# tphakala/birdnet-go

Measured on AMD Instinct MI355X. Metric: 3s-48kHz clips/sec (whole node) + max-abs prob diff vs TFLite, BirdNET v2.4, higher is better.
Workload: dtype f32; 1 GPU; BASELINE configs[1]: BirdNET v2.4 fp32, batch 256 x 3 s @ 48 kHz per GPU, mel front-end + CNN + head on device, raw logits out; batch_per_gpu=256, n_samples=144000, n_classes=6522, pipeline_depth=2, input_sets=4

## Files before the change

### birdnet-go_amd/csrc/engine.cpp

```cpp
#include "engine.h"

#include <algorithm>
#include <cmath>
#include <cstdio>
#include <cstdlib>
#include <cstring>
#include <mutex>
#include <sstream>

#include "../../include/bnhip.h"
#include "hostpipe.h"

namespace bnhip {

#define HIPCHK(call)                                                                           \
    do {                                                                                       \
        hipError_t e_ = (call);                                                                \
        if (e_ != hipSuccess) {                                                                \
            *err = std::string(#call) + ": " + hipGetErrorString(e_);                          \
            return false;                                                                      \
        }                                                                                      \
    } while (0)

Engine::~Engine() {
// ... 49 lines not shown
        if (steps[si].kind == S_FRONTEND) {
            specs[steps[si].spec].G = reinterpret_cast<const double*>(steps[si].w0);
            specs[steps[si].spec].window = steps[si].w1;
        }
        if (steps[si].kind == S_STFT) {
            specs[steps[si].spec].window_full = steps[si].w0;
            specs[steps[si].spec].bins = reinterpret_cast<const int*>(steps[si].w1);
            specs[steps[si].spec].stft_tw = reinterpret_cast<const double*>(steps[si].w2);
        }
    }
    HIPCHK(hipMalloc((void**)&d_stage_in, (size_t)max_batch * n_samples * 4));
    HIPCHK(hipMalloc((void**)&d_stage_logits, (size_t)max_batch * n_classes * 4));
    HIPCHK(hipMalloc((void**)&d_post_conf, (size_t)max_batch * n_classes * 4));
    if (emb_dim) HIPCHK(hipMalloc((void**)&d_stage_emb, (size_t)max_batch * emb_dim * 4));
    if (!defer_weights) mark_bf16_storage();
    if (autotune && !defer_weights) tune_or_load();
    *code = BNHIP_OK;
    return true;
}

namespace {
struct DevStreams { hipStream_t k[Engine::kMaxKStreams] = {nullptr, nullptr, nullptr, nullptr}; hipStream_t xfer = nullptr; int refs = 0; };
std::mutex g_ds_mu;
std::map<int, DevStreams> g_ds;
}

hipStream_t Engine::kernel_stream(int i) {
    if (i < 0 || i >= kMaxKStreams || device < 0) return nullptr;
    if (kstream[i]) return kstream[i];
    std::lock_guard<std::mutex> lk(g_ds_mu);
    DevStreams& ds = g_ds[device];
// ... 43 lines not shown
            if (!ctx_stream[c]) { ctx_stream[c] = kernel_stream(1 + c); if (!ctx_stream[c]) { *err = "hipStreamCreate failed"; return false; } }
            if (!ev_ctx_done[c]) HIPCHK(hipEventCreateWithFlags(&ev_ctx_done[c], hipEventDisableTiming));
        }
        if (!ctx_arena[c]) {
            if (c == 0) ctx_arena[c] = act_arena;
            else HIPCHK(hipMalloc((void**)&ctx_arena[c], std::max<size_t>(act_bytes, 256)));
        }
    }
    return true;
}

void Engine::finish_deferred() {
    if (device < 0) return;
    hipSetDevice(device);
    mark_bf16_storage();
    if (autotune) tune_or_load();
    defer_weights = false;
}

PwParams Engine::pw_params(const Step& s, int n, bool lane_tuning) const {
    PwParams p{nullptr, s.w0, s.w1, nullptr, nullptr, nullptr, n * s.H * s.W, s.Co, s.C, s.H * s.W, s.act, lane_tuning ? s.nt : s.nt_full,
               lane_tuning ? s.wm : s.wm_full};
    p.prec = precision; p.sw = pw_sw;
    p.a_bf16 = vals[s.in0].half ? 1 : 0; p.out_bf16 = vals[s.out].half ? 1 : 0;
    p.res_bf16 = (s.in2 >= 0 && vals[s.in2].half) ? 1 : 0;
    return p;
}
PwTail tail_of(const Step& s, const Step& c) {
    PwTail t;
    t.kind = s.tail; t.H = s.H; t.W = s.W;
    if (s.tail == 2) { t.k = c.kh; t.pt = c.pt; t.pl = c.pl; t.act = c.act; t.w = c.w0; t.bias = c.w1; }
// ... 19 lines not shown
        const Step& a = steps[si]; const Step& b = steps[si + 1];
        if (a.kind == S_MINMAX && b.kind == S_NORMALIZE && a.in0 == v_input && b.in0 == v_input && b.in1 == a.out) { norm_pair = si; break; }
    }
    if (norm_pair < 0 || !clip_norm_resident_fits(n_samples)) { norm_pair = -1; return; }
    pcm_direct = true;
    for (int si = 0; si < (int)steps.size(); si++) {
        if (si == norm_pair || si == norm_pair + 1) continue;
        const Step& s = steps[si];
        if (s.in0 == v_input || s.in1 == v_input || s.in2 == v_input) pcm_direct = false;
    }
}
bool Engine::norm_resident_taken(int n, const void* x, int bits, const float* xn) const {
    if (norm_pair < 0 || n <= 16) return false;
    const uintptr_t in_align = bits == 16 ? 8 : bits == 24 ? 4 : 16;
    return !(reinterpret_cast<uintptr_t>(x) & (in_align - 1)) && !(reinterpret_cast<uintptr_t>(xn) & 15);
}

float* Engine::vptr(int v, const float* d_in, float* d_logits, float* d_emb, int lane) const {
    if (v < 0) return nullptr;
    if (v == v_input) return const_cast<float*>(d_in);
    if (v == v_logits) return d_logits;
    if (part_hand && v == v_hand) return part_hand;
    (void)d_emb;
    char* base = cur_arena ? cur_arena : act_arena;
    if (lane >= 0) return reinterpret_cast<float*>(base + (size_t)lane * lane_bytes + vals[v].offset_lane);
    return reinterpret_cast<float*>(base + vals[v].offset);
}

hipEvent_t Engine::get_event() {
    if (!ev_pool.empty()) { hipEvent_t e = ev_pool.back(); ev_pool.pop_back(); return e; }
// ... 209 lines not shown
    for (int si = part_s0; si < s_end; si++) {
      for (int li = 0; li < nl; li++) {
        const Step& s = steps[si];
        const float* d_in = lanes[li].d_in; float* d_logits = lanes[li].d_logits; float* d_emb = lanes[li].d_emb;
        const int n = lanes[li].n, clip0 = nl > 1 ? li : -1;
        hipStream_t stream = lanes[li].st;
        float* in0 = vptr(s.in0, d_in, d_logits, d_emb, clip0);
        float* in1 = vptr(s.in1, d_in, d_logits, d_emb, clip0);
        float* in2 = vptr(s.in2, d_in, d_logits, d_emb, clip0);
        float* out = vptr(s.out, d_in, d_logits, d_emb, clip0);
        float* out2 = vptr(s.out2, d_in, d_logits, d_emb, clip0);
        if (s.kind == S_DW && si > 0 && steps[si - 1].tail == 2 && tail_taken(si - 1, n, nl > 1)) continue;
        if (s.kind == S_MEAN_PARTIAL && si > 0 && steps[si - 1].tail == 1 && tail_taken(si - 1, n, nl > 1)) continue;
        if (s.kind == S_MEAN_FINISH && si > 1 && steps[si - 2].tail == 1 && tail_taken(si - 2, n, nl > 1)) continue;
        if (s.kind == S_NORMALIZE && si == norm_pair + 1 && res_x[li]) continue;
        ProfEntry pe{};
        static const char* dbg_sync_before = getenv("BNHIP_DEBUG_SYNC_BEFORE");
        static const char* dbg_sync_after = getenv("BNHIP_DEBUG_SYNC_AFTER");
        static const char* dbg_ctx1_only = getenv("BNHIP_DEBUG_CTX1_ONLY");
        if (dbg_ctx1_only && cur_ctx == 1 && !strstr(dbg_ctx1_only, s.kclass)) continue;
        static const char* dbg_ctx1_skip = getenv("BNHIP_DEBUG_CTX1_SKIP");
        if (dbg_ctx1_skip && cur_ctx == 1 && strstr(dbg_ctx1_skip, s.kclass)) continue;
        if (dbg_sync_before && (!strcmp(dbg_sync_before, s.kclass) || s.name.rfind(dbg_sync_before, 0) == 0)) hipStreamSynchronize(stream);
        const bool prof_this = profiling && (profile_filter.empty() || profile_filter == s.kclass);
        if (prof_this) { pe.a = get_event(); pe.b = get_event(); pe.step = si; pe.n = n; hipEventRecord(pe.a, stream); }
        switch (s.kind) {
            case S_MINMAX:
                if (si == norm_pair && res_x[li]) {
                    const WinView lane_win = win_at(pcm.win, lanes[li].clip0);
                    if (!launch_clip_norm_resident(res_x[li], res_bits[li], n, n_samples, specs[0].eps, specs[0].norm_sub, specs[0].norm_mul,
// ... 79 lines not shown
                if (p.wm >= 13) p.wm = 10;
                if (p.wm >= 5 && s.wbx) launch_pw_bx3(p, s.wbx, stream);
                else launch_pw_gemm(p, stream);
                break;
            }
            case S_DW: {
                DwParams p = dw_params(s, in0, out, n);
                p.in_bf16 = vals[s.in0].half ? 1 : 0; p.out_bf16 = vals[s.out].half ? 1 : 0;
                if (s.dwl) launch_dwconv_lds(p, out2, s.shape, stream);
                else launch_dwconv(p, out2, stream);
                break;
            }
            case S_EXPAND_DW:
                {
                    StemGeom sg{s.H2, s.W2, s.pt2, s.pl2};
                    launch_expand_dw(in0, s.w0, s.w1, s.w2, s.w3, out, out2, n, s.H, s.W, s.C, s.Co,
                                     s.Ho, s.Wo, s.kh, s.sh, s.pt, s.pl, s.act, s.act2, s.shape, s.mode == 1 ? &sg : nullptr, stream,
                                     s.bx ? s.wbx : nullptr, precision, vals[s.out].half ? 1 : 0, vals[s.in0].half ? 1 : 0);
                }
                break;
            case S_MEAN_PARTIAL:
                launch_mean_partial(in0, out, n, s.H * s.W, s.C, s.S, stream);
                break;
            case S_MEAN_FINISH:
                launch_mean_finish(in0, out, n, s.H * s.W, s.C, s.S, stream);
                break;
            case S_SE: {
                SeParams p{in0, s.S, s.H * s.W, s.w0, s.w1, s.w2, s.w3, out, n, s.C, s.Cr, s.act, s.act2};
                if (cur_stream) p.threads = 256;
                launch_se(p, stream);
                break;
            }
            case S_UNARY:
// ... 176 lines not shown
```

### birdnet-go_amd/csrc/engine.h

```cpp
#pragma once
#include <hip/hip_runtime.h>

#include <map>
#include <string>
#include <vector>

#include "kernels.h"
#include "tflite_model.h"

namespace bnhip {

enum StepKind { S_MINMAX, S_FRONTEND, S_NORMALIZE, S_STFT, S_MELFIN, S_MELBAND, S_CONV_DIRECT, S_PW, S_DW, S_EXPAND_DW, S_MEAN_PARTIAL, S_MEAN_FINISH, S_SE, S_UNARY, S_BINARY,
                S_EW_UNARY, S_EW_BINARY, S_POOL, S_COPY, S_SOFTMAX, S_REDUCE, S_CONV_GENERIC,
                S_CONV_IGEMM };

struct GenGeom {
    int d[4] = {1, 1, 1, 1};
    long sa[4] = {0, 0, 0, 0}, sb[4] = {0, 0, 0, 0}, so[4] = {0, 0, 0, 0};
    long offa = 0, offo = 0;
    bool a_const = false, b_const = false;
    int mask = 0;
    float alpha = 0.f;
    bool fill = false;
    int dh = 1, dw = 1, depthwise = 0, mult = 1;
// ... 81 lines not shown
    int pw_sw = 0;
    bool use_graphs = false;
    void drop_graphs();
    static constexpr int kMaxDepth = 3;
    int depth = 1;
    hipStream_t ctx_stream[kMaxDepth] = {nullptr, nullptr, nullptr};
    char* ctx_arena[kMaxDepth] = {nullptr, nullptr, nullptr};
    static constexpr int kMinMaxScratch = 16 * (2 * kMinMaxParts + 2);
    float* mm_scratch = nullptr;
    bool mm_dirty = false;
    bool norm_resident = true;
    int norm_pair = -1;
    bool pcm_direct = false;
    void find_norm_pair();
    bool norm_resident_taken(int n, const void* x, int bits, const float* xn) const;
    hipEvent_t ev_ctx_fork = nullptr, ev_ctx_done[kMaxDepth] = {nullptr, nullptr, nullptr};
    unsigned call_idx = 0;
    bool run_pipelined(const float* d_in, int n, float* d_logits, float* d_emb, std::string* err);
    void sync_contexts();
    int host_depth = 2;
    bool ensure_contexts(int d, std::string* err, bool with_streams = true);
    bool run_on_context(int c, hipStream_t st, const float* d_in, int n, float* d_logits, float* d_emb, std::string* err, PcmSource pcm = {});
    int split_step = -1, v_hand = -1;
    float* d_hand = nullptr;
    std::vector<int> split_candidates;
    void pick_split();
    size_t hand_clip_bytes() const { return v_hand < 0 ? 0 : vals[v_hand].elems * (vals[v_hand].half ? 2 : 4); }
    bool ensure_hand(std::string* err);
    bool run_part(int c, hipStream_t st, int s0, int s1, const float* d_in, int n, float* hand, float* d_logits, float* d_emb, std::string* err, PcmSource pcm = {});
    int heatmap_pruned_step() const;
// ... 86 lines not shown
```

### birdnet-go_amd/csrc/expdw.hip

```cpp
#include "kernels.h"
#include "pw_common.h"

#include <algorithm>
#include <type_traits>
#include <cmath>
#include <cstdio>
#include <cstdlib>
#include <cstring>
#include <vector>

namespace bnhip {

struct ExpDwParams {
    const float* x; const float* we; const float* be; const float* wd; const float* bd;
    float* y; float* partial;
    int B, H, W, Cin, Cmid, Ho, Wo, pt, pl, act_e, act_d, tiles_h, tiles_w, cchunks, Kw, Cp;
    int Hin = 0, Win = 0, pts = 0, pls = 0;
    const uint16_t* wep = nullptr; int Kp = 0;
    int prec = 0;
    int xsh = 0, xsw = 1, ysh = 0, ysw = 1, tr = 0;
    int in_bf16 = 0, out_bf16 = 0;
    FDiv d_bpc{}, d_cch{}, d_tw{};
    int cpp = 0;
    FDiv d_part{};
};
#define ED_ES 36
#define ED_PERM2 0xfdce5764b98a1320ull
#define ED_PERM4 0xfdce9ba875461320ull
__device__ __forceinline__ int ed_perm(unsigned long long magic, int lane) {
    return (int)((magic >> ((lane >> 2) * 4)) & 15ull) * 4 + (lane & 3);
}
constexpr bool ed_perm_c4_rule(unsigned long long magic) {
    for (int g = 0; g < 16; g++)
        if (((magic >> (4 * g)) & 1ull) != (unsigned long long)((g >> 1) & 1)) return false;
    return true;
}
constexpr int expdw_min_waves(int K, int S, int TOW, int TRH) {
    const int tiw = (TOW - 1) * S + K, jt = (TRH * tiw + 15) / 16, jtw = (jt + 3) / 4;
    return jtw <= 4 ? 4 : (jtw == 5 ? 3 : 2);
// ... 340 lines not shown
            }
        }
    }
    if (tid < K * K * 8) wds[tid] = wdreg;
    __syncthreads();
    }

    const float4 sum = ed_phase2<K, S, TOH, TOW, TRH, 4>(p, E, wds, b, oh0, ow0, vr0, vr1, wave, tx, c4, n_base, bv, [] {});
    if (p.partial) {
        ed_sums_lanes(sum, red, wave, lane, c4);
        __syncthreads();
        ed_sums_out(p, red, tid, (size_t)b * tiles + tile, n_base);
    }
}

template <int K, int S, int TOH, int TOW, int TRH, bool STEM, int KW, bool LOOP = !STEM, int NW = 4, int PH = 0, int NS = 1>
__global__ __launch_bounds__(64 * NW, expdw_sk_waves(K, S, TOH, TOW, TRH, PH == 1 ? 16 * NS : KW, !LOOP, NW)) void k_expand_dw_sk(ExpDwParams p, unsigned nblk) {
    static_assert(PH == 0 || PH == 1, "phase 1 on the f32 or on the bf16 pipe");
    constexpr bool B16 = PH == 1;
    static_assert(!B16 || (LOOP && !STEM), "bf16 phase 1: chunk-loop form");
    static_assert(NS == 1 || B16, "several resident slabs: bf16 operands only");
    constexpr int KP = 32 * NS;
    static_assert(PH != 1 || KW == 24 || KW == 32, "one-product form: layers of the bf16 engines");
    static_assert(NW == 4 || (NW == 8 && LOOP && TOH % 8 == 0), "eight-wave blocks: chunk-loop form, tile height a multiple of 8");
    static_assert(KW == 16 || KW == 24 || KW == 32, "one or two K slabs, or a slab and a half");
    static_assert(!STEM || KW == 24, "the stem's window is 3 rows x 4 columns x 2 channels");
    constexpr int TIH = (TOH - 1) * S + K, TIW = (TOW - 1) * S + K;
    static_assert(TRH <= TIH, "TRH is a cap on the footprint rows");
    constexpr int NPIX = TRH * TIW, NPIXP = (NPIX + 15) / 16 * 16;
    constexpr int JT = NPIXP / 16, JTW = (JT + NW - 1) / NW;
    constexpr int SW = TOW / 8;
    constexpr int NMMA = B16 ? 2 * NS : KW / 2;
    __shared__ __attribute__((aligned(16))) float lds[NPIX * ED_ES + 64 * NW + K * K * 32];
// ... 31 lines not shown
    const int jtv = (nvalid + 15) >> 4;
    const int Cin = p.Cin;
    const int ncc = LOOP ? min(cpp, p.cchunks - cc0) : 1;
    const size_t tile_index = (size_t)b * tiles + tile;

    static_assert(SW * S == 2 || SW * S == 4, "lane permutation tables cover SW*S in {2, 4}");
    constexpr unsigned long long PERM = SW * S == 2 ? ED_PERM2 : ED_PERM4;
    const int pl = ed_perm(PERM, lane);
    const int c4 = pl & 7, tx = pl >> 3;

    bool xin[JTW];
    f32x4 xA[B16 ? 1 : JTW];
    f32x4 xB[(KW == 32 && !B16) ? JTW : 1];
    f32x2 xH[(KW == 24 && !B16) ? JTW : 1];
    bf16x8 xb[B16 ? JTW : 1][NS];
    auto load_x = [&]() {
        const float* xbase = STEM ? p.x + (size_t)b * p.Hin * p.Win * 2 : p.x;
#pragma unroll
        for (int a = 0; a < JTW; a++) {
            const int j = 16 * (wave + NW * a) + li;
            const int r = j / TIW, c = j - r * TIW;
            const int iw = iw0 + c;
            xin[a] = j < nvalid && iw >= 0 && iw < p.W;
            const int ihc = min(ih0 + vr0 + r, p.H - 1), iwc = min(max(iw, 0), p.W - 1);
            if constexpr (STEM) {
                const int row0 = ihc * 2 - p.pts, col0 = iwc * 2 - p.pls;
                auto tap2 = [&](int row, int col) {
                    const bool v = row >= 0 && row < p.Hin && col >= 0 && col < p.Win;
                    const float2 u = *reinterpret_cast<const float2*>(xbase + ((size_t)min(max(row, 0), p.Hin - 1) * p.Win + min(max(col, 0), p.Win - 1)) * 2);
                    return (f32x2){v ? u.x : 0.f, v ? u.y : 0.f};
                };
                const f32x2 u = tap2(row0 + (kq >> 1), col0 + (kq & 1) * 2), w = tap2(row0 + (kq >> 1), col0 + (kq & 1) * 2 + 1);
// ... 181 lines not shown
        }
        if (tid < K * K * 8) wds[tid] = q.wd;
        const float4 bv = q.bv;
        __syncthreads();
        if (LOOP && ci + 1 < ncc) fetch(cc + 1, q);

        const float4 sum = ed_phase2<K, S, TOH, TOW, TRH, NW>(p, E, wds, b, oh0, ow0, vr0, vr1, wave, tx, c4, n_base, bv, land);
        if (p.partial) ed_sums_lanes(sum, red, wave, lane, c4);
    }
    if (p.partial) {
        __syncthreads();
        ed_sums_out<NW>(p, red, tid, tile_index, (cc0 + ncc - 1) * 32);
    }
}

int expdw_kw(int Cin) { return (Cin & 1) ? (Cin + 15) / 16 * 16 : (Cin + 7) / 8 * 8; }
int expdw_skw(int Cin, int act_e, bool stem) {
    const int kw = expdw_kw(Cin);
    return !stem && act_e == ACT_SWISH && (kw == 16 || kw == 24 || kw == 32) ? kw : 0;
}
int expdw_cp(int Cmid) { return (Cmid + 31) / 32 * 32; }
struct ExpDwShape { int k, s, toh, tow, trh, nw = 4; };
static const ExpDwShape kExpDwShapes[] = {
    {3, 1, 8, 16, 10}, {3, 1, 4, 16, 6}, {3, 1, 8, 32, 6}, {3, 1, 8, 32, 10},
    {5, 1, 8, 16, 12}, {5, 1, 4, 16, 8}, {5, 1, 8, 32, 6}, {5, 1, 12, 16, 12},
    {3, 2, 4, 8, 9}, {3, 2, 8, 8, 12}, {3, 2, 8, 8, 17},
    {5, 2, 4, 8, 11}, {5, 2, 4, 16, 6}, {5, 2, 8, 8, 19},
    {3, 1, 8, 16, 10, 8}, {3, 1, 8, 32, 6, 8}, {3, 1, 8, 32, 10, 8}, {5, 1, 8, 16, 12, 8}, {5, 1, 8, 32, 6, 8},
    {3, 2, 8, 8, 12, 8}, {3, 2, 8, 8, 17, 8}, {5, 2, 8, 8, 19, 8},
};
// ... 90 lines not shown
        }
    return img;
}
bool expdw_sk_pipe16(int Cin, int act_e, bool stem, int prec, bool have_image) {
    static const bool off = getenv("BNHIP_EXPDW_B16") && atoi(getenv("BNHIP_EXPDW_B16")) == 0;
    static const int max_ns = getenv("BNHIP_EXPDW_B16_NS") ? atoi(getenv("BNHIP_EXPDW_B16_NS")) : 5;
    if (off || !have_image || stem || act_e != ACT_SWISH || !expdw_bx_ok(Cin)) return false;
    const int kw = expdw_skw(Cin, act_e, stem), ns = expdw_kp(Cin) / 32;
    return prec == 1 && ((kw == 24 || kw == 32) || (kw == 0 && (ns == 2 || ns == 3 || ns == 5) && ns <= max_ns));
}
bool expdw_supported(int k, int s, int Cin, int Cmid, int act_e, int prec) {
    if (!((k == 3 || k == 5) && (s == 1 || s == 2) && (Cin & 3) == 0 && (Cmid & 3) == 0)) return false;
    if (Cin <= 128) return true;
    return prec == 1 && expdw_sk_pipe16(Cin, act_e, false, prec, true);
}
template <int K, int S, int TH, int TW, int TR, bool H8, bool BX>
static void ed_launch(const ExpDwParams& p, unsigned nblk, hipStream_t st, bool fullw) {
    constexpr int VW = expdw_fullw_vw(K, S, TW);
    if constexpr (VW > 0) {
        if (fullw) {
            hipLaunchKernelGGL((k_expand_dw<K, S, TH, TW, TR, H8, BX, false, VW>), dim3(nblk), dim3(256), 0, st, p, nblk);
            return;
        }
    }
    hipLaunchKernelGGL((k_expand_dw<K, S, TH, TW, TR, H8, BX>), dim3(nblk), dim3(256), 0, st, p, nblk);
}
void launch_expand_dw(const float* x, const float* we, const float* be, const float* wd, const float* bd, float* y,
                      float* partial, int B, int H, int W, int Cin, int Cmid, int Ho, int Wo, int k, int s, int pt,
                      int pl, int act_e, int act_d, int shape, const StemGeom* stem, hipStream_t st, const uint16_t* wep, int prec, int out_bf16,
                      int in_bf16) {
    const bool pipe16 = expdw_sk_pipe16(Cin, act_e, stem != nullptr, prec, wep != nullptr);
    const ExpDwGeo g0{k, s, H, W, Ho, Wo, pt, pl, stem != nullptr, pipe16 ? 0 : expdw_skw(Cin, act_e, stem != nullptr)};
    if (!expdw_shape_fits(shape, g0, false)) shape = expdw_default_shape(g0);
    if (shape < 0) return;
    const ExpDwShape* sh = &kExpDwShapes[shape % kNumExpDwShapes];
    const bool tr = shape >= kNumExpDwShapes;
    const ExpDwGeo g = expdw_oriented(shape, g0);
    ExpDwParams p{x, we, be, wd, bd, y, partial, B, g.H, g.W, Cin, Cmid, g.Ho, g.Wo, g.pt, g.pl, act_e, act_d,
                  (g.Ho + sh->toh - 1) / sh->toh, (g.Wo + sh->tow - 1) / sh->tow, (Cmid + 31) / 32, expdw_kw(Cin), expdw_cp(Cmid)};
    p.xsh = tr ? 1 : W; p.xsw = tr ? W : 1; p.ysh = tr ? 1 : Wo; p.ysw = tr ? Wo : 1; p.tr = tr ? 1 : 0;
    p.out_bf16 = out_bf16;
    unsigned nblk = (unsigned)B * p.tiles_h * p.tiles_w * p.cchunks;
    p.d_bpc = make_fdiv((unsigned)(p.tiles_h * p.tiles_w * p.cchunks));
    p.d_cch = make_fdiv((unsigned)p.cchunks);
    p.d_tw = make_fdiv((unsigned)p.tiles_w);
    if (stem) p.Kw = 24;
    const bool sk = stem || pipe16 || (act_e == ACT_SWISH && (p.Kw == 16 || p.Kw == 24 || p.Kw == 32));
    const bool bx = wep != nullptr && !sk && expdw_bx_ok(Cin);
    if (bx) { p.wep = wep; p.Kp = expdw_kp(Cin); p.prec = prec; }
    const bool b16 = pipe16;
    const bool fullw = !sk && expdw_fullwidth(shape, g0);
    if (pipe16) { p.wep = wep; p.Kp = expdw_kp(Cin); p.prec = prec; p.in_bf16 = in_bf16; }
    if (sk && !stem) {
        const int tiles = p.tiles_h * p.tiles_w;
        nblk = (unsigned)B * tiles;
        p.d_bpc = make_fdiv((unsigned)tiles);
        const int cus = device_cus();
        if (p.cchunks > 1 && (long)B * tiles < cus / 2) {
            const int want = (int)std::min<long>(p.cchunks, (cus + (long)B * tiles - 1) / ((long)B * tiles));
            const int cpp = (p.cchunks + want - 1) / want, nparts = (p.cchunks + cpp - 1) / cpp;
            if (nparts > 1) {
                p.cpp = cpp;
                p.d_part = make_fdiv((unsigned)nparts);
                nblk = (unsigned)B * tiles * nparts;
                p.d_bpc = make_fdiv((unsigned)(tiles * nparts));
            }
        }
    }
    if (stem) {
        p.Hin = stem->Hin; p.Win = stem->Win; p.pts = stem->pt; p.pls = stem->pl;
#define ED_STEM(TH_, TW_, TR_)                                                                                \
    if (sh->k == 3 && sh->s == 1 && sh->toh == TH_ && sh->tow == TW_ && sh->trh == TR_) {                     \
        hipLaunchKernelGGL((k_expand_dw_sk<3, 1, TH_, TW_, TR_, true, 24>), dim3(nblk), dim3(256), 0, st, p, nblk);  \
        return;                                                                                               \
    }
        ED_STEM(8, 16, 10) ED_STEM(4, 16, 6) ED_STEM(8, 32, 6) ED_STEM(8, 32, 10)
#undef ED_STEM
        return;
    }
#define ED_CASE8(K_, S_, TH_, TW_, TR_)                                                                       \
    if (sh->nw == 8 && sh->k == K_ && sh->s == S_ && sh->toh == TH_ && sh->tow == TW_ && sh->trh == TR_) {    \
        if (p.Kw == 16) hipLaunchKernelGGL((k_expand_dw_sk<K_, S_, TH_, TW_, TR_, false, 16, true, 8>), dim3(nblk), dim3(512), 0, st, p, nblk); \
        else if (p.Kw == 24) hipLaunchKernelGGL((k_expand_dw_sk<K_, S_, TH_, TW_, TR_, false, 24, true, 8>), dim3(nblk), dim3(512), 0, st, p, nblk); \
        else hipLaunchKernelGGL((k_expand_dw_sk<K_, S_, TH_, TW_, TR_, false, 32, true, 8>), dim3(nblk), dim3(512), 0, st, p, nblk); \
        return;                                                                                               \
    }
    if (sh->nw == 8) {
        if (!sk || stem) return;
        ED_CASE8(3, 1, 8, 16, 10) ED_CASE8(3, 1, 8, 32, 6) ED_CASE8(3, 1, 8, 32, 10) ED_CASE8(5, 1, 8, 16, 12) ED_CASE8(5, 1, 8, 32, 6)
        ED_CASE8(3, 2, 8, 8, 12) ED_CASE8(3, 2, 8, 8, 17) ED_CASE8(5, 2, 8, 8, 19)
        return;
    }
#undef ED_CASE8
#define ED_CASE(K_, S_, TH_, TW_, TR_)                                                                        \
    if (sh->k == K_ && sh->s == S_ && sh->toh == TH_ && sh->tow == TW_ && sh->trh == TR_) {                   \
        if (bx) ed_launch<K_, S_, TH_, TW_, TR_, false, true>(p, nblk, st, fullw);                                \
        else if (b16 && p.Kp == 64) hipLaunchKernelGGL((k_expand_dw_sk<K_, S_, TH_, TW_, TR_, false, 32, true, 4, 1, 2>), dim3(nblk), dim3(256), 0, st, p, nblk); \
        else if (b16 && p.Kp == 96) hipLaunchKernelGGL((k_expand_dw_sk<K_, S_, TH_, TW_, TR_, false, 32, true, 4, 1, 3>), dim3(nblk), dim3(256), 0, st, p, nblk); \
        else if (b16 && p.Kp == 160) hipLaunchKernelGGL((k_expand_dw_sk<K_, S_, TH_, TW_, TR_, false, 32, true, 4, 1, 5>), dim3(nblk), dim3(256), 0, st, p, nblk); \
        else if (b16 && p.Kw == 24) hipLaunchKernelGGL((k_expand_dw_sk<K_, S_, TH_, TW_, TR_, false, 24, true, 4, 1>), dim3(nblk), dim3(256), 0, st, p, nblk); \
        else if (b16) hipLaunchKernelGGL((k_expand_dw_sk<K_, S_, TH_, TW_, TR_, false, 32, true, 4, 1>), dim3(nblk), dim3(256), 0, st, p, nblk); \
        else if (sk && p.Kw == 16) hipLaunchKernelGGL((k_expand_dw_sk<K_, S_, TH_, TW_, TR_, false, 16>), dim3(nblk), dim3(256), 0, st, p, nblk); \
        else if (sk && p.Kw == 24) hipLaunchKernelGGL((k_expand_dw_sk<K_, S_, TH_, TW_, TR_, false, 24>), dim3(nblk), dim3(256), 0, st, p, nblk); \
        else if (sk && p.Kw == 32) hipLaunchKernelGGL((k_expand_dw_sk<K_, S_, TH_, TW_, TR_, false, 32>), dim3(nblk), dim3(256), 0, st, p, nblk); \
        else if (p.Kw & 8) ed_launch<K_, S_, TH_, TW_, TR_, true, false>(p, nblk, st, fullw);                     \
        else ed_launch<K_, S_, TH_, TW_, TR_, false, false>(p, nblk, st, fullw);                                  \
        return;                                                                                               \
    }
    ED_CASE(3, 1, 8, 16, 10) ED_CASE(3, 1, 4, 16, 6) ED_CASE(3, 1, 8, 32, 6) ED_CASE(3, 1, 8, 32, 10)
    ED_CASE(5, 1, 8, 16, 12) ED_CASE(5, 1, 4, 16, 8) ED_CASE(5, 1, 8, 32, 6) ED_CASE(5, 1, 12, 16, 12)
    ED_CASE(3, 2, 4, 8, 9) ED_CASE(3, 2, 8, 8, 12) ED_CASE(3, 2, 8, 8, 17)
    ED_CASE(5, 2, 4, 8, 11) ED_CASE(5, 2, 4, 16, 6) ED_CASE(5, 2, 8, 8, 19)
#undef ED_CASE
}

bool dwconv_lds_supported(const DwParams& p) {
    return (p.C & 3) == 0 && p.kh == p.kw && p.sh == p.sw && (p.kh == 3 || p.kh == 5) && (p.sh == 1 || p.sh == 2);
}
void launch_dwconv_lds(const DwParams& q, float* partial, int shape, hipStream_t st) {
    const ExpDwGeo g0{q.kh, q.sh, q.H, q.W, q.Ho, q.Wo, q.pt, q.pl, false};
    if (!expdw_shape_fits(shape, g0, false)) shape = expdw_default_shape(g0);
    if (shape < 0) return;
    const ExpDwShape* sh = &kExpDwShapes[shape % kNumExpDwShapes];
    const bool tr = shape >= kNumExpDwShapes;
    const ExpDwGeo g = expdw_oriented(shape, g0);
    ExpDwParams p{q.in, nullptr, nullptr, q.w, q.bias, q.out, partial, q.B, g.H, g.W, q.C, q.C, g.Ho, g.Wo, g.pt, g.pl, ACT_NONE, q.act,
                  (g.Ho + sh->toh - 1) / sh->toh, (g.Wo + sh->tow - 1) / sh->tow, (q.C + 31) / 32, 0, q.C};
    p.xsh = tr ? 1 : q.W; p.xsw = tr ? q.W : 1; p.ysh = tr ? 1 : q.Wo; p.ysw = tr ? q.Wo : 1; p.tr = tr ? 1 : 0;
// ... 20 lines not shown
```

### birdnet-go_amd/csrc/kernels.h

```cpp
#pragma once
#include <atomic>
#include <hip/hip_runtime.h>

#include <vector>
#include <cstdint>

#include "analyze.h"

namespace bnhip {

inline int device_cus() {
    static std::atomic<int> cus[64];
    int dev = 0;
    if (hipGetDevice(&dev) != hipSuccess) { (void)hipGetLastError(); return 256; }
    if (dev < 0 || dev >= 64) return 256;
    int c = cus[dev].load(std::memory_order_relaxed);
    if (c > 0) return c;
    hipDeviceProp_t pr{};
    if (hipGetDeviceProperties(&pr, dev) != hipSuccess || pr.multiProcessorCount <= 0) { (void)hipGetLastError(); return 256; }
    cus[dev].store(pr.multiProcessorCount, std::memory_order_relaxed);
    return pr.multiProcessorCount;
}

struct PwGrid { int nblk_n; unsigned nblk; };
// ... 160 lines not shown

bool expdw_supported(int k, int s, int Cin, int Cmid, int act_e = 0, int prec = 0);
struct ExpDwGeo { int k, s, H, W, Ho, Wo, pt, pl; bool stem = false; int skw = 0; };
int expdw_skw(int Cin, int act_e, bool stem);
bool expdw_sk_pipe16(int Cin, int act_e, bool stem, int prec, bool have_image);
int expdw_sum_slabs(const ExpDwGeo& g);
int expdw_num_shapes();
bool expdw_shape_fits(int idx, const ExpDwGeo& g, bool planning = true);
int expdw_shape_slabs(int idx, const ExpDwGeo& g);
bool expdw_fullwidth(int idx, const ExpDwGeo& g);
int expdw_default_shape(const ExpDwGeo& g);
int expdw_max_slabs(const ExpDwGeo& g);
struct StemGeom { int Hin, Win, pt, pl; };
int expdw_kw(int Cin);
int expdw_cp(int Cmid);
void launch_expand_dw(const float* x, const float* we, const float* be, const float* wd, const float* bd, float* y,
                      float* partial, int B, int H, int W, int Cin, int Cmid, int Ho, int Wo, int k, int s, int pt,
                      int pl, int act_e, int act_d, int shape ,
                      const StemGeom* stem ,
                      hipStream_t st, const uint16_t* wep = nullptr ,
                      int prec = 0 ,
                      int out_bf16 = 0 ,
                      int in_bf16 = 0 );
bool dwconv_lds_supported(const DwParams& p);
void launch_dwconv_lds(const DwParams& p, float* partial, int shape, hipStream_t st);
bool expdw_bx_ok(int Cin);
int expdw_kp(int Cin);
std::vector<uint16_t> expdw_bx_image(const float* We , int Cmid, int Cin);

int mean_splits(int HW);
int mean_partial_py(int C);
void launch_mean_partial(const float* in, float* partial, int B, int HW, int C, int S, hipStream_t s);
void launch_mean_finish(const float* partial, float* out, int B, int HW, int C, int S, hipStream_t s);

struct SeParams {
    const float* partial; int S; int HW;
    const float* w1; const float* b1;
    const float* w2; const float* b2;
// ... 50 lines not shown
```

### birdnet-go_amd/csrc/planner.cpp

```cpp
#include "engine.h"

#include <algorithm>
#include <cmath>
#include <cstdio>
#include <cstdlib>
#include <cstring>
#include <map>

#include "../../include/bnhip.h"

namespace bnhip {

namespace {

size_t align_up(size_t v, size_t a) { return (v + a - 1) / a * a; }

struct Planner {
    const TflModel& m;
    std::vector<int> producer;
    std::vector<std::vector<int>> consumers;
    std::vector<int> uses;
    std::vector<char> absorbed;
    std::string err;

// ... 1432 lines not shown
        int want_wm = 0, want_nt = 6;
        if (const char* e = getenv("BNHIP_PW_TAIL_FORM")) { if (sscanf(e, "%d,%d", &want_wm, &want_nt) != 2) { want_wm = 0; want_nt = 6; } }
        int fit = 0, forced_fit = 0;
        for (int wm : {14, 13, 15}) if (pw_tail_ok(p, t, 6, wm)) { if (!fit) fit = wm; if (wm == want_wm && pw_tail_ok(p, t, want_nt, wm)) forced_fit = wm; }
        if (!fit) continue;
        s.tail = t.kind;
        if (pw_sw & PW_SW_TAIL_FORCE) { s.wm = s.wm_full = forced_fit ? forced_fit : fit; s.nt = s.nt_full = forced_fit ? want_nt : 6; }
    }
}

bool Engine::build(TflModel m, int dev, int maxb, bool plan_only, std::string* err, int* code) {
    device = dev;
    max_batch = maxb;
    pw_sw = pw_switches_from_env();
    if (const char* e = getenv("BNHIP_NORM_RESIDENT")) norm_resident = atoi(e) != 0;
    const PlanSwitches sw;
    *code = BNHIP_E_UNSUPPORTED;
    if (!run_graph_passes(&m, err)) return false;
    if (!select_outputs(m, &logits_output, &embedding_output)) {
        *code = BNHIP_E_INVALID;
        *err = "logits_output / embedding_output do not name two distinct graph outputs";
        return false;
    }
    Lowering L(*this, m, sw);
    if (!L.input_values() || !L.match_frontends() || !L.frontend() || !L.ops() || !L.bind_outputs()) {
        *err = L.err; *code = L.code;
        return false;
    }
    tensor_value = L.tv;
    mark_tails();
    find_norm_pair();

    mark_liveness(vals, steps);
    if (v_emb >= 0) vals[v_emb].last = (int)steps.size();
    for (const Value& v : vals)
        if (v.elems * (size_t)max_batch >= ((size_t)1 << 31)) {
            *err = "max_batch too large for this model: a " + std::to_string(v.elems) + "-element activation times " +
                   std::to_string(max_batch) + " clips exceeds 32-bit indexing";
            *code = BNHIP_E_INVALID;
            return false;
        }
    n_lanes = std::max(1, std::min(n_lanes, kMaxLanes));
    lane_cap = (max_batch + n_lanes - 1) / n_lanes;
    act_bytes = plan_arena(vals, steps, (size_t)max_batch, false, no_reuse);
    lane_bytes = n_lanes > 1 ? align_up(plan_arena(vals, steps, (size_t)lane_cap, true, no_reuse), 256) : 0;
    act_bytes = std::max(act_bytes, lane_bytes * (size_t)n_lanes);
    pick_split();

    w_bytes = L.w.img.size() * sizeof(float);
    if (plan_only) { device = -1; *code = BNHIP_OK; return true; }
    return bind_device(L.w, err, code);
}

}
```

### birdnet-go_amd/csrc/tune.cpp

```cpp
#include "engine.h"

#include <algorithm>
#include <cstdio>
#include <cstdlib>
#include <cstring>
#include <mutex>
#include <sstream>

namespace bnhip {

bool Engine::expdw_pipe16(const Step& s) const {
    return s.kind == S_EXPAND_DW && expdw_sk_pipe16(s.C, s.act, s.mode == 1, precision, s.bx && s.wbx != nullptr && bf16x3);
}
ExpDwGeo Engine::expdw_geo(const Step& s) const {
    const bool fused = s.kind == S_EXPAND_DW, stem = fused && s.mode == 1;
    return ExpDwGeo{s.kh, s.sh, s.H, s.W, s.Ho, s.Wo, s.pt, s.pl, stem, (fused && !expdw_pipe16(s)) ? expdw_skw(s.C, s.act, stem) : 0};
}
void Engine::set_sum_slabs(Step& s, int S) {
    s.S = S;
    for (auto& c : steps) if (&c != &s && c.in0 == s.out2) c.S = S;
}
static bool pw_padding_ok(int Co, int nt) {
    const long cols = (long)((Co + nt * 16 - 1) / (nt * 16)) * nt * 16;
    return cols * 100 <= (long)((Co + 15) / 16 * 16) * 130;
// ... 350 lines not shown
                    if (wm == 11) {
                        if (nt != 1 || !pw_b16s_ok(p)) continue;
                    }
                    if (wm == 12) {
                        if (by_work) continue;
                        if ((nt != 4 && nt != 6 && nt != 8) || !pw_ws_ok(p) || !pw_ws_fills(p)) continue;
                        if (precision == 1 && nt != 4) continue;
                    }
                    const float ms = timer.back_to_back([&]() { launch_pw_bx3(p, s.wbx, stream); });
                    if (getenv("BNHIP_DEBUG")) fprintf(stderr, "[bnhip] tune %-16s n=%d M=%d N=%d K=%d nt=%d wm=%d (bf16x3): %.1f us (%.1f TF fp32-equivalent)\n", s.name.c_str(), n, p.M, s.Co, s.C, nt, wm, ms * 1e3, flops / (ms * 1e-3) / 1e12);
                    if (ms < bbest * 0.98f) { bbest = ms; best_nt = nt; best_wm = wm; }
                }
        }
        nt_out = best_nt; wm_out = best_wm;
    });
}

void Engine::autotune_tail() {
    LaunchTimer timer(stream);
    const bool forced = (pw_sw & PW_SW_TAIL_FORCE) != 0;
    tune_lane_then_full(*this, [&](size_t si, int n, bool lane, int& nt_out, int& wm_out) {
        const Step& s = steps[si];
        if (s.kind != S_PW || !s.tail || !s.wbx) return;
        Step& c = steps[si + 1];
        PwParams p = pw_params(s, n, lane);
        if (p.wm >= 13) { p.wm = 6; p.nt = 0; }
        p.A = vptr(s.in0, d_stage_in, d_stage_logits, nullptr);
        p.out = vptr(s.out, d_stage_in, d_stage_logits, nullptr);
        PwTail t = tail_of(s, c);
        float* mean_out = nullptr;
// ... 34 lines not shown
```

Baseline: 81300 clips/s.

## Fold small pointwise projection into following stride-2 expand-depthwise kernel

Detects a narrow pointwise conv (K≤32, N≤16, no activation or residual) whose only reader is a stride-2 3x3 expand-depthwise block. It then computes the projection inside the expand-dw kernel with f32 MFMA while loading the input tile, which removes one launch and the write and re-read of the intermediate activation. Input lifetimes are extended so the arena planner keeps them alive. An autotune step times the pair against the folded kernel and falls back to the pair if folding is slower. The cost is that each overlapping input tile reads more channels and recomputes the projection at halo positions.

```diff
diff --git a/birdnet-go_amd/csrc/engine.cpp b/birdnet-go_amd/csrc/engine.cpp
--- a/birdnet-go_amd/csrc/engine.cpp
+++ b/birdnet-go_amd/csrc/engine.cpp
@@ -87,7 +87,7 @@
     HIPCHK(hipMalloc((void**)&d_post_conf, (size_t)max_batch * n_classes * 4));
     if (emb_dim) HIPCHK(hipMalloc((void**)&d_stage_emb, (size_t)max_batch * emb_dim * 4));
     if (!defer_weights) mark_bf16_storage();
-    if (autotune && !defer_weights) tune_or_load();
+    if (autotune && !defer_weights) { tune_or_load(); time_fold_proj(); }
     *code = BNHIP_OK;
     return true;
 }
@@ -161,7 +161,7 @@
     if (device < 0) return;
     hipSetDevice(device);
     mark_bf16_storage();
-    if (autotune) tune_or_load();
+    if (autotune) { tune_or_load(); time_fold_proj(); }
     defer_weights = false;
 }
 
@@ -211,6 +211,34 @@
     if (norm_pair < 0 || n <= 16) return false;
     const uintptr_t in_align = bits == 16 ? 8 : bits == 24 ? 4 : 16;
     return !(reinterpret_cast<uintptr_t>(x) & (in_align - 1)) && !(reinterpret_cast<uintptr_t>(xn) & 15);
+}
+
+void Engine::find_fold_pair() {
+    fold_pair = -1;
+    if (!fold_proj || precision != 0) return;
+    const int ns = (int)steps.size();
+    for (int si = 0; si + 1 < ns; si++) {
+        const Step& a = steps[si]; const Step& b = steps[si + 1];
+        if (a.kind != S_PW || b.kind != S_EXPAND_DW || b.mode == 1 || b.in0 != a.out || a.out < 0) continue;
+        if (a.in2 >= 0 || a.act != ACT_NONE || a.tail || (a.bx && bf16x3) || a.Co > 16 || a.C > 32 || (a.C & 3) || (a.Co & 3)) continue;
+        if (a.H != b.H || a.W != b.W || a.Co != b.C || b.kh != 3 || b.sh != 2 || expdw_skw(b.C, b.act, false) != 16) continue;
+        if (a.out == v_logits || a.out == v_emb || a.out == v_input || vals[a.out].external) continue;
+        int readers = 0;
+        for (const Step& t : steps)
+            for (int v : {t.in0, t.in1, t.in2}) readers += v == a.out;
+        if (readers != 1) continue;
+        fold_pair = si;
+        break;
+    }
+}
+bool Engine::fold_taken(int si, int n, bool lane_tuning) const {
+    if (fold_pair < 0 || si != fold_pair || !fold_faster) return false;
+    const int s_end = part_s1 < 0 ? (int)steps.size() : part_s1;
+    if (si < part_s0 || si + 1 >= s_end) return false;
+    const Step& a = steps[si]; const Step& b = steps[si + 1];
+    if (a.wbx && (lane_tuning ? a.wm : a.wm_full) >= 5) return false;
+    if (vals[a.in0].half || vals[a.out].half || vals[b.out].half || expdw_pipe16(b)) return false;
+    return expdw_proj_ok(b.shape, expdw_geo(b), n, b.Co);
 }
 
 float* Engine::vptr(int v, const float* d_in, float* d_logits, float* d_emb, int lane) const {
@@ -450,6 +478,7 @@
         if (s.kind == S_MEAN_PARTIAL && si > 0 && steps[si - 1].tail == 1 && tail_taken(si - 1, n, nl > 1)) continue;
         if (s.kind == S_MEAN_FINISH && si > 1 && steps[si - 2].tail == 1 && tail_taken(si - 2, n, nl > 1)) continue;
         if (s.kind == S_NORMALIZE && si == norm_pair + 1 && res_x[li]) continue;
+        if (s.kind == S_PW && fold_taken(si, n, nl > 1)) continue;
         ProfEntry pe{};
         static const char* dbg_sync_before = getenv("BNHIP_DEBUG_SYNC_BEFORE");
         static const char* dbg_sync_after = getenv("BNHIP_DEBUG_SYNC_AFTER");
@@ -559,9 +588,18 @@
             case S_EXPAND_DW:
                 {
                     StemGeom sg{s.H2, s.W2, s.pt2, s.pl2};
-                    launch_expand_dw(in0, s.w0, s.w1, s.w2, s.w3, out, out2, n, s.H, s.W, s.C, s.Co,
-                                     s.Ho, s.Wo, s.kh, s.sh, s.pt, s.pl, s.act, s.act2, s.shape, s.mode == 1 ? &sg : nullptr, stream,
-                                     s.bx ? s.wbx : nullptr, precision, vals[s.out].half ? 1 : 0, vals[s.in0].half ? 1 : 0);
+                    ExpDwProj pj{};
+                    const bool fold = si > 0 && fold_taken(si - 1, n, nl > 1);
+                    if (fold) {
+                        const Step& a = steps[si - 1];
+                        pj = ExpDwProj{vptr(a.in0, d_in, d_logits, d_emb, clip0), a.w0, a.w1, vptr(a.in1, d_in, d_logits, d_emb, clip0), a.C, a.Co};
+                        pe.more_bytes = 4.0 * s.H * s.W * (a.C - a.Co) + (a.in1 >= 0 ? 4.0 * a.C : 0.0);
+                    }
+                    if (!launch_expand_dw(in0, s.w0, s.w1, s.w2, s.w3, out, out2, n, s.H, s.W, s.C, s.Co,
+                                          s.Ho, s.Wo, s.kh, s.sh, s.pt, s.pl, s.act, s.act2, s.shape, s.mode == 1 ? &sg : nullptr, stream,
+                                          s.bx ? s.wbx : nullptr, precision, vals[s.out].half ? 1 : 0, vals[s.in0].half ? 1 : 0, fold ? &pj : nullptr)) {
+                        *err = "k_expand_dw_sk refused a folded projection its predicate accepted"; mm_dirty = true; return false;
+                    }
                 }
                 break;
             case S_MEAN_PARTIAL:
diff --git a/birdnet-go_amd/csrc/engine.h b/birdnet-go_amd/csrc/engine.h
--- a/birdnet-go_amd/csrc/engine.h
+++ b/birdnet-go_amd/csrc/engine.h
@@ -119,6 +119,13 @@
     bool pcm_direct = false;
     void find_norm_pair();
     bool norm_resident_taken(int n, const void* x, int bits, const float* xn) const;
+    bool fold_proj = true;
+    int fold_pair = -1;
+    bool fold_faster = true;
+    float fold_us[2] = {0.f, 0.f};
+    void find_fold_pair();
+    bool fold_taken(int si, int n, bool lane_tuning) const;
+    void time_fold_proj();
     hipEvent_t ev_ctx_fork = nullptr, ev_ctx_done[kMaxDepth] = {nullptr, nullptr, nullptr};
     unsigned call_idx = 0;
     bool run_pipelined(const float* d_in, int n, float* d_logits, float* d_emb, std::string* err);
diff --git a/birdnet-go_amd/csrc/expdw.hip b/birdnet-go_amd/csrc/expdw.hip
--- a/birdnet-go_amd/csrc/expdw.hip
+++ b/birdnet-go_amd/csrc/expdw.hip
@@ -23,6 +23,8 @@
     FDiv d_bpc{}, d_cch{}, d_tw{};
     int cpp = 0;
     FDiv d_part{};
+    const float* pj_w = nullptr; const float* pj_b = nullptr; const float* pj_gate = nullptr;
+    int pj_K = 0, pj_N = 0;
 };
 #define ED_ES 36
 #define ED_PERM2 0xfdce5764b98a1320ull
@@ -393,9 +395,10 @@
     }
 }
 
-template <int K, int S, int TOH, int TOW, int TRH, bool STEM, int KW, bool LOOP = !STEM, int NW = 4, int PH = 0, int NS = 1>
-__global__ __launch_bounds__(64 * NW, expdw_sk_waves(K, S, TOH, TOW, TRH, PH == 1 ? 16 * NS : KW, !LOOP, NW)) void k_expand_dw_sk(ExpDwParams p, unsigned nblk) {
+template <int K, int S, int TOH, int TOW, int TRH, bool STEM, int KW, bool LOOP, int NW, int PH, int NS, bool PROJ>
+__device__ __forceinline__ void expand_dw_sk_body(ExpDwParams p, unsigned nblk) {
     static_assert(PH == 0 || PH == 1, "phase 1 on the f32 or on the bf16 pipe");
+    static_assert(!PROJ || (LOOP && !STEM && PH == 0 && KW == 16), "folded projection: chunk-loop form on the f32 pipe, one K slab");
     constexpr bool B16 = PH == 1;
     static_assert(!B16 || (LOOP && !STEM), "bf16 phase 1: chunk-loop form");
     static_assert(NS == 1 || B16, "several resident slabs: bf16 operands only");
@@ -457,8 +460,56 @@
     f32x4 xB[(KW == 32 && !B16) ? JTW : 1];
     f32x2 xH[(KW == 24 && !B16) ? JTW : 1];
     bf16x8 xb[B16 ? JTW : 1][NS];
+    f32x4 pjw0 = {0.f, 0.f, 0.f, 0.f}, pjw1 = pjw0, pjb = pjw0, pjg0 = {1.f, 1.f, 1.f, 1.f}, pjg1 = pjg0;
+    const bool pjk0 = PROJ && 4 * kq < p.pj_K, pjk1 = PROJ && 16 + 4 * kq < p.pj_K;
+    if constexpr (PROJ) {
+        auto ld4 = [](const float* q) { const float4 t = *reinterpret_cast<const float4*>(q); return (f32x4){t.x, t.y, t.z, t.w}; };
+        if (li < p.pj_N && pjk0) pjw0 = ld4(p.pj_w + li * p.pj_K + 4 * kq);
+        if (li < p.pj_N && pjk1) pjw1 = ld4(p.pj_w + li * p.pj_K + 16 + 4 * kq);
+        if (p.pj_b && 4 * kq < p.pj_N) pjb = ld4(p.pj_b + 4 * kq);
+        if (p.pj_gate) {
+            const float* gq = p.pj_gate + (size_t)b * p.pj_K;
+            pjg0 = ld4(gq + (pjk0 ? 4 * kq : 0));
+            pjg1 = ld4(gq + (pjk1 ? 16 + 4 * kq : 0));
+        }
+    }
     auto load_x = [&]() {
         const float* xbase = STEM ? p.x + (size_t)b * p.Hin * p.Win * 2 : p.x;
+        if constexpr (PROJ) {
+            const f32x4 z = {0.f, 0.f, 0.f, 0.f};
+            f32x4 y0[JTW], y1[JTW];
+#pragma unroll
+            for (int a = 0; a < JTW; a++) {
+                const int j = 16 * (wave + NW * a) + li;
+                const int r = j / TIW, c = j - r * TIW;
+                const int iw = iw0 + c;
+                xin[a] = j < nvalid && iw >= 0 && iw < p.W;
+                const int ihc = min(ih0 + vr0 + r, p.H - 1), iwc = min(max(iw, 0), p.W - 1);
+                const float* xp = xbase + (size_t)((b * p.H * p.W + ihc * p.xsh + iwc * p.xsw) * p.pj_K);
+                const float4 t = *reinterpret_cast<const float4*>(xp + (pjk0 ? 4 * kq : 0));
+                const float4 t2 = *reinterpret_cast<const float4*>(xp + (pjk1 ? 16 + 4 * kq : 0));
+                y0[a] = (f32x4){t.x, t.y, t.z, t.w}; y1[a] = (f32x4){t2.x, t2.y, t2.z, t2.w};
+            }
+#pragma unroll
+            for (int a = 0; a < JTW; a++) {
+                f32x4 s0 = y0[a], s1 = y1[a];
+                if (p.pj_gate) {
+                    s0[0] *= pjg0[0]; s0[1] *= pjg0[1]; s0[2] *= pjg0[2]; s0[3] *= pjg0[3];
+                    s1[0] *= pjg1[0]; s1[1] *= pjg1[1]; s1[2] *= pjg1[2]; s1[3] *= pjg1[3];
+                }
+                s0 = pjk0 ? s0 : z; s1 = pjk1 ? s1 : z;
+                f32x4 d = z;
+                if (wave + NW * a < jtv) {
+#pragma unroll
+                    for (int sidx = 0; sidx < 4; sidx++) d = __builtin_amdgcn_mfma_f32_16x16x4f32(pjw0[sidx], s0[sidx], d, 0, 0, 0);
+#pragma unroll
+                    for (int sidx = 0; sidx < 4; sidx++) d = __builtin_amdgcn_mfma_f32_16x16x4f32(pjw1[sidx], s1[sidx], d, 0, 0, 0);
+                    if (p.pj_b) d += pjb;
+                }
+                xA[a] = d;
+            }
+            return;
+        }
 #pragma unroll
         for (int a = 0; a < JTW; a++) {
             const int j = 16 * (wave + NW * a) + li;
@@ -670,6 +721,15 @@
     }
 }
 
+template <int K, int S, int TOH, int TOW, int TRH, bool STEM, int KW, bool LOOP = !STEM, int NW = 4, int PH = 0, int NS = 1>
+__global__ __launch_bounds__(64 * NW, expdw_sk_waves(K, S, TOH, TOW, TRH, PH == 1 ? 16 * NS : KW, !LOOP, NW)) void k_expand_dw_sk(ExpDwParams p, unsigned nblk) {
+    expand_dw_sk_body<K, S, TOH, TOW, TRH, STEM, KW, LOOP, NW, PH, NS, false>(p, nblk);
+}
+template <int K, int S, int TOH, int TOW, int TRH, int NW>
+__global__ __launch_bounds__(64 * NW, expdw_sk_waves(K, S, TOH, TOW, TRH, 16, false, NW)) void k_expand_dw_sk_proj(ExpDwParams p, unsigned nblk) {
+    expand_dw_sk_body<K, S, TOH, TOW, TRH, false, 16, true, NW, 0, 1, true>(p, nblk);
+}
+
 int expdw_kw(int Cin) { return (Cin & 1) ? (Cin + 15) / 16 * 16 : (Cin + 7) / 8 * 8; }
 int expdw_skw(int Cin, int act_e, bool stem) {
     const int kw = expdw_kw(Cin);
@@ -790,6 +850,23 @@
     if (Cin <= 128) return true;
     return prec == 1 && expdw_sk_pipe16(Cin, act_e, false, prec, true);
 }
+static int expdw_cut_cpp(int B, int tiles, int cchunks) {
+    const int cus = device_cus();
+    if (cchunks <= 1 || (long)B * tiles >= cus / 2) return 0;
+    const int want = (int)std::min<long>(cchunks, (cus + (long)B * tiles - 1) / ((long)B * tiles));
+    const int cpp = (cchunks + want - 1) / want, nparts = (cchunks + cpp - 1) / cpp;
+    return nparts > 1 ? cpp : 0;
+}
+bool expdw_proj_ok(int shape, const ExpDwGeo& g0, int B, int Cmid) {
+    if (g0.stem || g0.skw != 16) return false;
+    if (!expdw_shape_fits(shape, g0, false)) shape = expdw_default_shape(g0);
+    if (shape < 0) return false;
+    const ExpDwShape& sh = kExpDwShapes[shape % kNumExpDwShapes];
+    if (sh.k != 3 || sh.s != 2) return false;
+    const ExpDwGeo g = expdw_oriented(shape, g0);
+    const int tiles = ((g.Ho + sh.toh - 1) / sh.toh) * ((g.Wo + sh.tow - 1) / sh.tow);
+    return expdw_cut_cpp(B, tiles, (Cmid + 31) / 32) == 0;
+}
 template <int K, int S, int TH, int TW, int TR, bool H8, bool BX>
 static void ed_launch(const ExpDwParams& p, unsigned nblk, hipStream_t st, bool fullw) {
     constexpr int VW = expdw_fullw_vw(K, S, TW);
@@ -801,18 +878,19 @@
     }
     hipLaunchKernelGGL((k_expand_dw<K, S, TH, TW, TR, H8, BX>), dim3(nblk), dim3(256), 0, st, p, nblk);
 }
-void launch_expand_dw(const float* x, const float* we, const float* be, const float* wd, const float* bd, float* y,
+bool launch_expand_dw(const float* x, const float* we, const float* be, const float* wd, const float* bd, float* y,
                       float* partial, int B, int H, int W, int Cin, int Cmid, int Ho, int Wo, int k, int s, int pt,
                       int pl, int act_e, int act_d, int shape, const StemGeom* stem, hipStream_t st, const uint16_t* wep, int prec, int out_bf16,
-                      int in_bf16) {
+                      int in_bf16, const ExpDwProj* proj) {
     const bool pipe16 = expdw_sk_pipe16(Cin, act_e, stem != nullptr, prec, wep != nullptr);
     const ExpDwGeo g0{k, s, H, W, Ho, Wo, pt, pl, stem != nullptr, pipe16 ? 0 : expdw_skw(Cin, act_e, stem != nullptr)};
+    if (proj && (pipe16 || out_bf16 || in_bf16 || proj->N != Cin || proj->K > 32 || (proj->K & 3) || (proj->N & 3) || !expdw_proj_ok(shape, g0, B, Cmid))) return false;
     if (!expdw_shape_fits(shape, g0, false)) shape = expdw_default_shape(g0);
-    if (shape < 0) return;
+    if (shape < 0) return true;
     const ExpDwShape* sh = &kExpDwShapes[shape % kNumExpDwShapes];
     const bool tr = shape >= kNumExpDwShapes;
     const ExpDwGeo g = expdw_oriented(shape, g0);
-    ExpDwParams p{x, we, be, wd, bd, y, partial, B, g.H, g.W, Cin, Cmid, g.Ho, g.Wo, g.pt, g.pl, act_e, act_d,
+    ExpDwParams p{proj ? proj->x : x, we, be, wd, bd, y, partial, B, g.H, g.W, Cin, Cmid, g.Ho, g.Wo, g.pt, g.pl, act_e, act_d,
                   (g.Ho + sh->toh - 1) / sh->toh, (g.Wo + sh->tow - 1) / sh->tow, (Cmid + 31) / 32, expdw_kw(Cin), expdw_cp(Cmid)};
     p.xsh = tr ? 1 : W; p.xsw = tr ? W : 1; p.ysh = tr ? 1 : Wo; p.ysw = tr ? Wo : 1; p.tr = tr ? 1 : 0;
     p.out_bf16 = out_bf16;
@@ -831,16 +909,12 @@
         const int tiles = p.tiles_h * p.tiles_w;
         nblk = (unsigned)B * tiles;
         p.d_bpc = make_fdiv((unsigned)tiles);
-        const int cus = device_cus();
-        if (p.cchunks > 1 && (long)B * tiles < cus / 2) {
-            const int want = (int)std::min<long>(p.cchunks, (cus + (long)B * tiles - 1) / ((long)B * tiles));
-            const int cpp = (p.cchunks + want - 1) / want, nparts = (p.cchunks + cpp - 1) / cpp;
-            if (nparts > 1) {
-                p.cpp = cpp;
-                p.d_part = make_fdiv((unsigned)nparts);
-                nblk = (unsigned)B * tiles * nparts;
-                p.d_bpc = make_fdiv((unsigned)(tiles * nparts));
-            }
+        if (const int cpp = expdw_cut_cpp(B, tiles, p.cchunks)) {
+            const int nparts = (p.cchunks + cpp - 1) / cpp;
+            p.cpp = cpp;
+            p.d_part = make_fdiv((unsigned)nparts);
+            nblk = (unsigned)B * tiles * nparts;
+            p.d_bpc = make_fdiv((unsigned)(tiles * nparts));
         }
     }
     if (stem) {
@@ -848,24 +922,36 @@
 #define ED_STEM(TH_, TW_, TR_)                                                                                \
     if (sh->k == 3 && sh->s == 1 && sh->toh == TH_ && sh->tow == TW_ && sh->trh == TR_) {                     \
         hipLaunchKernelGGL((k_expand_dw_sk<3, 1, TH_, TW_, TR_, true, 24>), dim3(nblk), dim3(256), 0, st, p, nblk);  \
-        return;                                                                                               \
+        return true;                                                                                          \
     }
         ED_STEM(8, 16, 10) ED_STEM(4, 16, 6) ED_STEM(8, 32, 6) ED_STEM(8, 32, 10)
 #undef ED_STEM
-        return;
-    }
-#define ED_CASE8(K_, S_, TH_, TW_, TR_)                                                                       \
+        return true;
+    }
+    if (proj) {
+        if (!sk || p.Kw != 16 || p.cpp != 0) return false;
+        p.pj_w = proj->w; p.pj_b = proj->bias; p.pj_gate = proj->gate; p.pj_K = proj->K; p.pj_N = proj->N;
+#define ED_PROJ(TH_, TW_, TR_, NW_)                                                                           \
+    if (sh->nw == NW_ && sh->toh == TH_ && sh->tow == TW_ && sh->trh == TR_) {                                \
+        hipLaunchKernelGGL((k_expand_dw_sk_proj<3, 2, TH_, TW_, TR_, NW_>), dim3(nblk), dim3(64 * NW_), 0, st, p, nblk); \
+        return true;                                                                                          \
+    }
+        ED_PROJ(4, 8, 9, 4) ED_PROJ(8, 8, 12, 4) ED_PROJ(8, 8, 17, 4) ED_PROJ(8, 8, 12, 8) ED_PROJ(8, 8, 17, 8)
+#undef ED_PROJ
+        return false;
+    }
+#define ED_CASE8(K_, S_, TH_, TW_, TR_)                                                                     \
     if (sh->nw == 8 && sh->k == K_ && sh->s == S_ && sh->toh == TH_ && sh->tow == TW_ && sh->trh == TR_) {    \
         if (p.Kw == 16) hipLaunchKernelGGL((k_expand_dw_sk<K_, S_, TH_, TW_, TR_, false, 16, true, 8>), dim3(nblk), dim3(512), 0, st, p, nblk); \
         else if (p.Kw == 24) hipLaunchKernelGGL((k_expand_dw_sk<K_, S_, TH_, TW_, TR_, false, 24, true, 8>), dim3(nblk), dim3(512), 0, st, p, nblk); \
         else hipLaunchKernelGGL((k_expand_dw_sk<K_, S_, TH_, TW_, TR_, false, 32, true, 8>), dim3(nblk), dim3(512), 0, st, p, nblk); \
-        return;                                                                                               \
+        return true;                                                                                          \
     }
     if (sh->nw == 8) {
-        if (!sk || stem) return;
+        if (!sk || stem) return true;
         ED_CASE8(3, 1, 8, 16, 10) ED_CASE8(3, 1, 8, 32, 6) ED_CASE8(3, 1, 8, 32, 10) ED_CASE8(5, 1, 8, 16, 12) ED_CASE8(5, 1, 8, 32, 6)
         ED_CASE8(3, 2, 8, 8, 12) ED_CASE8(3, 2, 8, 8, 17) ED_CASE8(5, 2, 8, 8, 19)
-        return;
+        return true;
     }
 #undef ED_CASE8
 #define ED_CASE(K_, S_, TH_, TW_, TR_)                                                                        \
@@ -881,13 +967,14 @@
         else if (sk && p.Kw == 32) hipLaunchKernelGGL((k_expand_dw_sk<K_, S_, TH_, TW_, TR_, false, 32>), dim3(nblk), dim3(256), 0, st, p, nblk); \
         else if (p.Kw & 8) ed_launch<K_, S_, TH_, TW_, TR_, true, false>(p, nblk, st, fullw);                     \
         else ed_launch<K_, S_, TH_, TW_, TR_, false, false>(p, nblk, st, fullw);                                  \
-        return;                                                                                               \
+        return true;                                                                                          \
     }
     ED_CASE(3, 1, 8, 16, 10) ED_CASE(3, 1, 4, 16, 6) ED_CASE(3, 1, 8, 32, 6) ED_CASE(3, 1, 8, 32, 10)
     ED_CASE(5, 1, 8, 16, 12) ED_CASE(5, 1, 4, 16, 8) ED_CASE(5, 1, 8, 32, 6) ED_CASE(5, 1, 12, 16, 12)
     ED_CASE(3, 2, 4, 8, 9) ED_CASE(3, 2, 8, 8, 12) ED_CASE(3, 2, 8, 8, 17)
     ED_CASE(5, 2, 4, 8, 11) ED_CASE(5, 2, 4, 16, 6) ED_CASE(5, 2, 8, 8, 19)
 #undef ED_CASE
+    return true;
 }
 
 bool dwconv_lds_supported(const DwParams& p) {
diff --git a/birdnet-go_amd/csrc/kernels.h b/birdnet-go_amd/csrc/kernels.h
--- a/birdnet-go_amd/csrc/kernels.h
+++ b/birdnet-go_amd/csrc/kernels.h
@@ -198,14 +198,17 @@
 struct StemGeom { int Hin, Win, pt, pl; };
 int expdw_kw(int Cin);
 int expdw_cp(int Cmid);
-void launch_expand_dw(const float* x, const float* we, const float* be, const float* wd, const float* bd, float* y,
+struct ExpDwProj { const float* x; const float* w; const float* bias; const float* gate; int K, N; };
+bool expdw_proj_ok(int shape, const ExpDwGeo& g, int B, int Cmid);
+bool launch_expand_dw(const float* x, const float* we, const float* be, const float* wd, const float* bd, float* y,
                       float* partial, int B, int H, int W, int Cin, int Cmid, int Ho, int Wo, int k, int s, int pt,
                       int pl, int act_e, int act_d, int shape ,
                       const StemGeom* stem ,
                       hipStream_t st, const uint16_t* wep = nullptr ,
                       int prec = 0 ,
                       int out_bf16 = 0 ,
-                      int in_bf16 = 0 );
+                      int in_bf16 = 0 ,
+                      const ExpDwProj* proj = nullptr );
 bool dwconv_lds_supported(const DwParams& p);
 void launch_dwconv_lds(const DwParams& p, float* partial, int shape, hipStream_t st);
 bool expdw_bx_ok(int Cin);
diff --git a/birdnet-go_amd/csrc/planner.cpp b/birdnet-go_amd/csrc/planner.cpp
--- a/birdnet-go_amd/csrc/planner.cpp
+++ b/birdnet-go_amd/csrc/planner.cpp
@@ -1470,6 +1470,7 @@
     max_batch = maxb;
     pw_sw = pw_switches_from_env();
     if (const char* e = getenv("BNHIP_NORM_RESIDENT")) norm_resident = atoi(e) != 0;
+    if (const char* e = getenv("BNHIP_FOLD_PROJ")) fold_proj = atoi(e) != 0;
     const PlanSwitches sw;
     *code = BNHIP_E_UNSUPPORTED;
     if (!run_graph_passes(&m, err)) return false;
@@ -1486,6 +1487,7 @@
     tensor_value = L.tv;
     mark_tails();
     find_norm_pair();
+    find_fold_pair();
 
     mark_liveness(vals, steps);
     if (v_emb >= 0) vals[v_emb].last = (int)steps.size();
@@ -1498,9 +1500,15 @@
         }
     n_lanes = std::max(1, std::min(n_lanes, kMaxLanes));
     lane_cap = (max_batch + n_lanes - 1) / n_lanes;
+    const int fv0 = fold_pair >= 0 ? steps[fold_pair].in0 : -1, fv1 = fold_pair >= 0 ? steps[fold_pair].in1 : -1;
+    const int fl0 = fv0 >= 0 ? vals[fv0].last : 0, fl1 = fv1 >= 0 ? vals[fv1].last : 0;
+    if (fv0 >= 0) vals[fv0].last = std::max(fl0, fold_pair + 1);
+    if (fv1 >= 0) vals[fv1].last = std::max(fl1, fold_pair + 1);
     act_bytes = plan_arena(vals, steps, (size_t)max_batch, false, no_reuse);
     lane_bytes = n_lanes > 1 ? align_up(plan_arena(vals, steps, (size_t)lane_cap, true, no_reuse), 256) : 0;
     act_bytes = std::max(act_bytes, lane_bytes * (size_t)n_lanes);
+    if (fv0 >= 0) vals[fv0].last = fl0;
+    if (fv1 >= 0) vals[fv1].last = fl1;
     pick_split();
 
     w_bytes = L.w.img.size() * sizeof(float);
diff --git a/birdnet-go_amd/csrc/tune.cpp b/birdnet-go_amd/csrc/tune.cpp
--- a/birdnet-go_amd/csrc/tune.cpp
+++ b/birdnet-go_amd/csrc/tune.cpp
@@ -388,6 +388,30 @@
         }
         nt_out = best_nt; wm_out = best_wm;
     });
+}
+
+void Engine::time_fold_proj() {
+    fold_faster = true; fold_us[0] = fold_us[1] = 0.f;
+    if (fold_pair < 0 || device < 0) return;
+    const int n = max_batch;
+    if (!fold_taken(fold_pair, n, false)) return;
+    const Step& a = steps[fold_pair]; const Step& b = steps[fold_pair + 1];
+    PwParams p = pw_params(a, n, false);
+    p.A = vptr(a.in0, d_stage_in, d_stage_logits, nullptr); p.ascale = vptr(a.in1, d_stage_in, d_stage_logits, nullptr);
+    p.out = vptr(a.out, d_stage_in, d_stage_logits, nullptr);
+    float* out = vptr(b.out, d_stage_in, d_stage_logits, nullptr);
+    float* out2 = vptr(b.out2, d_stage_in, d_stage_logits, nullptr);
+    const ExpDwProj pj{p.A, a.w0, a.w1, p.ascale, a.C, a.Co};
+    auto expdw = [&](const ExpDwProj* proj) {
+        launch_expand_dw(p.out, b.w0, b.w1, b.w2, b.w3, out, out2, n, b.H, b.W, b.C, b.Co, b.Ho, b.Wo, b.kh, b.sh, b.pt, b.pl, b.act, b.act2,
+                         b.shape, nullptr, stream, nullptr, precision, 0, 0, proj);
+    };
+    LaunchTimer timer(stream);
+    const float pair = timer.back_to_back([&]() { launch_pw_gemm(p, stream); expdw(nullptr); });
+    const float fold = timer.back_to_back([&]() { expdw(&pj); });
+    fold_us[0] = pair * 1e3f; fold_us[1] = fold * 1e3f;
+    fold_faster = fold < pair;
+    if (getenv("BNHIP_DEBUG")) fprintf(stderr, "[bnhip] tune %s + %s: pair %.1f us, one launch %.1f us -> %s\n", a.name.c_str(), b.name.c_str(), pair * 1e3, fold * 1e3, fold_faster ? "folded" : "pair");
 }
 
 void Engine::autotune_tail() {
```

Result: faster. 82970 clips/s (median of 6 runs) (+2.1%).
